# PlasmaControl/spectrogram-enhancement

Measured on AMD Instinct MI355X. Metric: spectrograms/s (STFT+VAE-denoise fwd) at 1/2/4/8 GPUs; PSNR vs CPU ref, higher is better.
Workload: dtype fp16; 1 GPU; BASELINE config 5 per GPU: end-to-end STFT -> SVD -> autoencoder-denoise inference stream, 16,512-sample fp16 shots -> specgr 128x128 (256 hann / hop 128) -> denoiseSignal default -> 3-layer conv AE (16/32/64, 5x5) fp16 forward -> fp16 reconstructions (32,768 B per shot); shots_per_launch=2048, samples=16512, stft_dtype=fp32, svd_dtype=fp32 (fp64 small algebra), ae_dtype=fp16, parallelism=shot-sharded x1, streams_per_gpu=2

## Files before the change

### spectrogram-enhancement_amd/csrc/conv_rows.hip

```cpp
#include <hip/hip_runtime.h>

#include <algorithm>
#include <cstdint>
#include <string>
#include <type_traits>

#include "lds_dma.hpp"
#include "specenh.h"
#include "runtime.hpp"
#include "wave.hpp"

namespace specenh {

namespace {

typedef _Float16 f16x8 __attribute__((ext_vector_type(8)));
typedef __bf16 bf16x8 __attribute__((ext_vector_type(8)));
typedef float f32x4 __attribute__((ext_vector_type(4)));

template <typename T>
__device__ __forceinline__ f32x4 mfma(const uint4& a, const uint4& b, f32x4 acc) {
  if constexpr (__is_same(T, _Float16))
    return __builtin_amdgcn_mfma_f32_16x16x32_f16(__builtin_bit_cast(f16x8, a),
                                                  __builtin_bit_cast(f16x8, b), acc, 0, 0, 0);
// ... 1209 lines not shown
  static constexpr int LDS = RING * ROWB;
  static constexpr int DMA_WAVES = W * CI * 2 / 1024;
  static_assert(WAVES == 4 && DMA_WAVES <= WAVES && (W * CI * 2) % 1024 == 0, "shape");
  static_assert(tap(3, DY0, DY0) || tap(0, DY0, DY0) || any_tap(DY0, 0), "neighbourhood");
};

__device__ __forceinline__ int x32off(int ps, int g) { return ps * 64 + 16 * (g ^ ((ps >> 1) & 3)); }

template <typename T, int CO, int W, int K, int LEAD>
__global__ __launch_bounds__((TC32<CO, W, K>::THREADS)) __attribute__((amdgpu_waves_per_eu(2)))
void convt_rows32_kernel(CRArgs a) {
  using C = TC32<CO, W, K>;
  constexpr int DY0 = C::DY0, DY1 = C::DY1, NDY = C::NDY;
  static_assert(LEAD >= 1 && NDY + LEAD + 1 <= C::RING, "ring: positions g .. g + NDY + LEAD live");
  extern __shared__ __attribute__((aligned(16))) unsigned char ring[];
  const int tid = threadIdx.x, lane = tid & 63;
  const int wv = __builtin_amdgcn_readfirstlane(tid >> 6);
  const int m = lane & 15, kg = lane >> 4;
  const int wx = wv % C::NWIN, nb = wv / C::NWIN;
  const int H = a.H, SPI = H + C::GAP;
  const int G = gridDim.x;
  const int nimg = ((int)a.N - (int)blockIdx.x + G - 1) / G;
  const int S = nimg * SPI;

  {
    uint4* z = reinterpret_cast<uint4*>(ring);
    for (int e = tid; e < C::LDS / 16; e += C::THREADS) z[e] = uint4{0u, 0u, 0u, 0u};
  }
  uint4 wf[K * K];
  {
    const T* __restrict__ Wg = reinterpret_cast<const T*>(a.w);
#pragma unroll
    for (int ph = 0; ph < 4; ++ph)
#pragma unroll
      for (int dy = DY0; dy <= DY1; ++dy)
#pragma unroll
        for (int dx = DY0; dx <= DY1; ++dx)
          if (C::tap(ph, dy, dx))
            wf[C::tap_index(ph, dy, dx)] = *reinterpret_cast<const uint4*>(
                Wg + (((16 * nb + m) * K + C::ky_of(ph >> 1, dy)) * K + C::ky_of(ph & 1, dx)) * 32 +
                8 * kg);
  }
  const f32x4 bias = f32x4{a.b[16 * nb + 4 * kg], a.b[16 * nb + 4 * kg + 1],
                           a.b[16 * nb + 4 * kg + 2], a.b[16 * nb + 4 * kg + 3]};
  resident_loads_landed();
  int xo[NDY];
#pragma unroll
  for (int dx = DY0; dx <= DY1; ++dx) xo[dx - DY0] = x32off(16 * wx + m + dx - DY0, kg);
  const T* __restrict__ X = reinterpret_cast<const T*>(a.x);
  const bool dma_wave = wv < C::DMA_WAVES;
  int dsrc = 0;
  if (dma_wave) {
    const int c = 64 * wv + lane;
    const int x = c / 4, gs = c & 3, ps = x - DY0;
    dsrc = x * 32 + 8 * (gs ^ ((ps >> 1) & 3));
  }
  auto stage_at = [&](int p, int il, int r) -> bool {
    if (!dma_wave) return false;
    unsigned char* dst = ring + (p & 7) * C::ROWB + (-DY0) * 64 + 1024 * wv;
    if (il < nimg && r >= 0 && r < H) {
      const long long n = (long long)blockIdx.x + (long long)il * G;
      lds_dma16_s(X + ((n * H + r) * W) * 32, 2u * dsrc, dst);
      return true;
    }
    *reinterpret_cast<uint4*>(dst + 16 * lane) = uint4{0u, 0u, 0u, 0u};
    return false;
  };
  auto stage = [&](int p) -> bool {
    const int il = p / SPI;
    return stage_at(p, il, p - il * SPI + DY0);
  };
  __syncthreads();
#pragma unroll
  for (int p = 0; p < NDY + LEAD; ++p) stage(p);
  asm volatile("s_waitcnt vmcnt(0)" ::: "memory");
  lds_barrier();

  T* __restrict__ O = reinterpret_cast<T*>(a.out);
  const int OW = 2 * W;
  uint2 pk[4];
  long long po = 0;
  bool held = false;
  int vmn = 0;
  int mk[LEAD + 1];
#pragma unroll
  for (int i = 0; i <= LEAD; ++i) mk[i] = -1;
  auto store_held = [&]() {
    if (held) {
#pragma unroll
      for (int ph = 0; ph < 4; ++ph)
        gstore8(O + po + ((ph >> 1) * OW + (ph & 1)) * CO, pk[ph]);
      vmn += 4;
    }
  };
  int il = 0, s = 0;
  int ilp = (NDY + LEAD) / SPI, sp = NDY + LEAD - ilp * SPI;
  for (int g = 0; g < S; ++g) {
    store_held();
    held = false;
    mk[LEAD] = stage_at(g + NDY + LEAD, ilp, sp + DY0) ? ++vmn : -1;
    if (s < H) {
      f32x4 acc[4] = {bias, bias, bias, bias};
#pragma unroll
      for (int dy = DY0; dy <= DY1; ++dy) {
        const unsigned char* src = ring + ((g + dy - DY0) & 7) * C::ROWB;
#pragma unroll
        for (int dx = DY0; dx <= DY1; ++dx) {
          if (!C::any_tap(dy, dx)) continue;
          const uint4 b = *reinterpret_cast<const uint4*>(src + xo[dx - DY0]);
#pragma unroll
          for (int ph = 0; ph < 4; ++ph)
            if (C::tap(ph, dy, dx)) acc[ph] = mfma<T>(wf[C::tap_index(ph, dy, dx)], b, acc[ph]);
        }
      }
#pragma unroll
      for (int ph = 0; ph < 4; ++ph) pk[ph] = relu_pack4<T>(acc[ph]);
      const long long n = (long long)blockIdx.x + (long long)il * G;
      po = ((n * 2 * H + 2 * s) * OW + 2 * (16 * wx + m)) * CO + 16 * nb + 4 * kg;
      held = true;
    }
    if (mk[0] >= 0) wait_vmcnt_ss<15>(vmn - mk[0]);
    lds_barrier();
#pragma unroll
    for (int i = 0; i < LEAD; ++i) mk[i] = mk[i + 1];
    if (++s == SPI) { s = 0; ++il; }
    if (++sp == SPI) { sp = 0; ++ilp; }
  }
  store_held();
}

template <typename T, int CO, int W, int K>
hipError_t launch_convt_rows32(const CRArgs& a, hipStream_t st) {
  using C = TC32<CO, W, K>;
  constexpr int LEAD = 8 - C::NDY - 1 < 3 ? 8 - C::NDY - 1 : 3;
  const void* k = reinterpret_cast<const void*>(&convt_rows32_kernel<T, CO, W, K, LEAD>);
  static int per_cu[64] = {};
  int dev = 0;
  hipError_t e = hipGetDevice(&dev);
  if (e != hipSuccess) return e;
  if (dev < 0 || dev >= 64) dev = 0;
  if (per_cu[dev] == 0) {
    int pc = 0;
    e = hipOccupancyMaxActiveBlocksPerMultiprocessor(&pc, k, C::THREADS, C::LDS);
    if (e != hipSuccess) return e;
    per_cu[dev] = std::max(1, pc);
  }
  const long long grid = std::min<long long>(a.N, (long long)per_cu[dev] * device_cus());
  SPECENH_LAUNCH((convt_rows32_kernel<T, CO, W, K, LEAD>), dim3((unsigned)grid),
                 dim3(C::THREADS), C::LDS, st, a);
  return hipGetLastError();
}

constexpr int C1W = 128;
constexpr int C1CW = 72;
constexpr int C1ROW = 2 * C1CW;
constexpr int C1RING = 16;
constexpr int C1LDS = C1RING * C1ROW * 4;

template <typename T>
__global__ __launch_bounds__(256) void conv1_rows_pool_kernel(CRArgs a) {
  extern __shared__ __attribute__((aligned(16))) unsigned char ring_raw[];
  uint32_t* const ring = reinterpret_cast<uint32_t*>(ring_raw);
  const int tid = threadIdx.x, lane = tid & 63;
  const int wv = __builtin_amdgcn_readfirstlane(tid >> 6);
  const int m = lane & 15, kg = lane >> 4;
  const int H = a.H, SPI = H / 2 + 2, PPI = H + 4;
  const int G = gridDim.x;
  const int nimg = ((int)a.N - (int)blockIdx.x + G - 1) / G;
  const int S = nimg * SPI;

  for (int e = tid; e < C1RING * C1ROW; e += 256) ring[e] = 0u;
  uint4 w0, w1;
  {
    const T* __restrict__ Wg = reinterpret_cast<const T*>(a.w);
    uint32_t q0[4], q1[4];
#pragma unroll
    for (int i = 0; i < 4; ++i) {
      float v[4];
#pragma unroll
      for (int h = 0; h < 2; ++h) {
        const int kx = 2 * i + h;
        v[2 * h] = kx < 5 ? (float)Wg[(m * 5 + kg) * 5 + kx] : 0.f;
        v[2 * h + 1] = kx < 5 && kg == 0 ? (float)Wg[(m * 5 + 4) * 5 + kx] : 0.f;
      }
      q0[i] = pack2<T>(v[0], v[2]);
      q1[i] = pack2<T>(v[1], v[3]);
    }
    w0 = uint4{q0[0], q0[1], q0[2], q0[3]};
    w1 = uint4{q1[0], q1[1], q1[2], q1[3]};
  }
  const f32x4 bias = f32x4{a.b[4 * kg], a.b[4 * kg + 1], a.b[4 * kg + 2], a.b[4 * kg + 3]};

  const T* __restrict__ X = reinterpret_cast<const T*>(a.x);
  auto stage = [&](int pp) -> int {
    if (wv != 0) return 0;
    int nd = 0;
#pragma unroll
    for (int j = 0; j < 2; ++j) {
      const int pos = pp + j;
      const int il = pos / PPI, r = pos - il * PPI - 2;
      uint32_t* dst = ring + (pos & (C1RING - 1)) * C1ROW + 4;
      if (il < nimg && r >= 0 && r < H) {
        const long long n = (long long)blockIdx.x + (long long)il * G;
        if (lane < 16) lds_dma16(X + (n * H + r) * C1W + 8 * lane, dst);
        ++nd;
      } else if (lane < 16) {
        *reinterpret_cast<uint4*>(dst + 4 * lane) = uint4{0u, 0u, 0u, 0u};
      }
    }
    return nd;
  };
  auto shift = [&](int pp) {
    if (tid < 2 * C1CW) {
      const int j = tid / C1CW, i = tid - j * C1CW;
      uint32_t* row = ring + ((pp + j) & (C1RING - 1)) * C1ROW;
      const uint32_t lo = row[i], hi = row[i + 1];
      row[C1CW + i] = __builtin_amdgcn_alignbit(hi, lo, 16);
    }
  };
  __syncthreads();
  for (int pp = 0; pp < 10; pp += 2) stage(pp);
  asm volatile("s_waitcnt vmcnt(0)" ::: "memory");
  lds_barrier();
  shift(0); shift(2); shift(4);
  lds_barrier();

  const int wbase = 16 * wv + m + 3;
  auto bfrag = [&](int pos, int cb) -> uint4 {
    const uint32_t* row = ring + ((pos + kg) & (C1RING - 1)) * C1ROW + cb * C1CW + wbase;
    return uint4{row[0], row[1], row[2], row[3]};
  };
  T* __restrict__ O = reinterpret_cast<T*>(a.out);
  const int PW = C1W / 2, PH = H / 2;
  for (int g = 0; g < S; ++g) {
    const int nd = stage(2 * g + 10);
    shift(2 * g + 6);
    const int il = g / SPI, p = g - il * SPI;
    if (p < PH) {
      const int pb = 2 * g;
      f32x4 acc[2][2];
#pragma unroll
      for (int dy = 0; dy < 2; ++dy)
#pragma unroll
        for (int cb = 0; cb < 2; ++cb) {
          const uint4 b = bfrag(pb + dy, cb);
          uint4 b4 = bfrag(pb + dy + 4, cb);
          if (kg != 0) b4 = uint4{0u, 0u, 0u, 0u};
          acc[dy][cb] = mfma<T>(w0, b, bias);
          acc[dy][cb] = mfma<T>(w1, b4, acc[dy][cb]);
        }
      float v[4];
#pragma unroll
      for (int i = 0; i < 4; ++i)
        v[i] = fmaxf(fmaxf(fmaxf(acc[0][0][i], acc[0][1][i]), fmaxf(acc[1][0][i], acc[1][1][i])),
                     0.f);
      const long long n = (long long)blockIdx.x + (long long)il * G;
      *reinterpret_cast<uint2*>(O + ((n * PH + p) * PW + 16 * wv + m) * 16 + 4 * kg) =
          uint2{pack2<T>(v[0], v[1]), pack2<T>(v[2], v[3])};
    }
    if (wv == 0) {
      const int younger = nd + (p < PH ? 1 : 0);
      if (younger == 0) asm volatile("s_waitcnt vmcnt(0)" ::: "memory");
      else if (younger == 1) asm volatile("s_waitcnt vmcnt(1)" ::: "memory");
      else if (younger == 2) asm volatile("s_waitcnt vmcnt(2)" ::: "memory");
      else asm volatile("s_waitcnt vmcnt(3)" ::: "memory");
    }
    lds_barrier();
  }
}

template <typename T>
hipError_t launch_conv1_rows(const CRArgs& a, hipStream_t st) {
  const void* k = reinterpret_cast<const void*>(&conv1_rows_pool_kernel<T>);
  static int per_cu[64] = {};
  int dev = 0;
  hipError_t e = hipGetDevice(&dev);
  if (e != hipSuccess) return e;
  if (dev < 0 || dev >= 64) dev = 0;
  if (per_cu[dev] == 0) {
    int pc = 0;
    e = hipOccupancyMaxActiveBlocksPerMultiprocessor(&pc, k, 256, C1LDS);
    if (e != hipSuccess) return e;
    per_cu[dev] = std::max(1, pc);
  }
  const long long grid = std::min<long long>(a.N, (long long)per_cu[dev] * device_cus());
  SPECENH_LAUNCH(conv1_rows_pool_kernel<T>, dim3((unsigned)grid), dim3(256), C1LDS, st, a);
  return hipGetLastError();
}

struct E2Args {
  const void* x;
  const void* w1;
  const float* b1;
  const void* w2;
  const float* b2;
  void* out;
  int N, H;
};

constexpr int E2R1 = 32;
#ifndef SPECENH_ENC2_COPIES
#define SPECENH_ENC2_COPIES 4
#endif
constexpr int E2NC = SPECENH_ENC2_COPIES;
__host__ __device__ constexpr int E2CB(int c) {
  return E2NC == 4 ? (c == 0 ? 0 : c == 1 ? 72 : c == 2 ? 178 : 250) : c * C1CW;
}
constexpr int E2ROW = E2NC == 4 ? 352 : 2 * C1CW;
constexpr int E2RROWS = E2R1 + 2;
#ifndef SPECENH_ENC2_STAGGER
#define SPECENH_ENC2_STAGGER 0
#endif

constexpr int E2LDS = RC<16, 32, 64>::LDS + E2RROWS * E2ROW * 4 + 48 * 4;
constexpr int E2TILE = 32 * 32 * 2;
constexpr int E2LDS1 = E2LDS + 2 * E2TILE;
__host__ __device__ constexpr int e2_tile_write(int p, int c8) {
  return 64 * p + 8 * (c8 ^ (2 * ((p >> 1) & 3)));
}
__host__ __device__ constexpr int e2_tile_read(int k, int l) {
  const int p = 16 * k + (l >> 2);
  return 64 * p + 16 * ((l & 3) ^ ((p >> 1) & 3));
}

__device__ __forceinline__ uint32_t max_s16x2(uint32_t x, uint32_t y) {
  typedef short s2 __attribute__((ext_vector_type(2)));
  return __builtin_bit_cast(uint32_t, __builtin_elementwise_max(__builtin_bit_cast(s2, x),
                                                                __builtin_bit_cast(s2, y)));
}

template <typename T, int WPE, int SCHED = 0>
__global__ __launch_bounds__(512) __attribute__((amdgpu_waves_per_eu(WPE)))
void enc2_rows_kernel(E2Args a) {
  static_assert(SCHED == 0 || (SCHED == 1 && WPE == 4), "schedule");
  using C = RC<16, 32, 64>;
  extern __shared__ __attribute__((aligned(16))) unsigned char lds[];
  unsigned char* const ring = lds;
  uint32_t* const ring1 = reinterpret_cast<uint32_t*>(lds + C::LDS);
  const int tid = threadIdx.x, lane = tid & 63;
  const int wv = __builtin_amdgcn_readfirstlane(tid >> 6);
  const int m = lane & 15, kg = lane >> 4;
  const int wx = wv % C::NWIN, nb = wv / C::NWIN;
  const int x0 = 16 * wx;
  const int H1 = a.H, H = H1 / 2;
  const int SPI = H / 2 + 1, PPI = H1 + 4;
  const int G = gridDim.x;
  const int nimg = ((int)a.N - (int)blockIdx.x + G - 1) / G;
  const int S = nimg * SPI + 1;

  for (int e = tid; e < (C::LDS + E2RROWS * E2ROW * 4) / 16; e += 512)
    reinterpret_cast<uint4*>(lds)[e] = uint4{0u, 0u, 0u, 0u};
  float* const btab = reinterpret_cast<float*>(lds + C::LDS + E2RROWS * E2ROW * 4);
  if (tid < 16) btab[tid] = a.b1[tid];
  else if (tid < 48) btab[tid] = a.b2[tid - 16];
  auto bias2_ld = [&]() { return *reinterpret_cast<const f32x4*>(btab + 16 + 16 * nb + 4 * kg); };

  uint4 wf[13];
  {
    const T* __restrict__ Wg = reinterpret_cast<const T*>(a.w2);
    const int co = 16 * nb + m, hi = kg >> 1, c8 = 8 * (kg & 1);
    auto tap = [&](int ky, int kx) {
      return *reinterpret_cast<const uint4*>(Wg + ((co * 5 + ky) * 5 + kx) * 16 + c8);
    };
#pragma unroll
    for (int ky = 0; ky < 5; ++ky) {
      wf[ky] = tap(ky, hi);
      wf[5 + ky] = tap(ky, 2 + hi);
    }
    wf[10] = tap(hi, 4);
    wf[11] = tap(2 + hi, 4);
    wf[12] = hi ? uint4{0u, 0u, 0u, 0u} : tap(4, 4);
  }

  const int boff = (x0 + m + (kg >> 1)) * 32 + 16 * (kg & 1);
  const int fo = (x0 + m + 4) * 32 + 16 * (kg & 1);
  const int foff = fo + (kg >> 1) * C::ROWB, foffw = fo - (kg >> 1) * 7 * C::ROWB;

  uint4 v0, v1;
  {
    const T* __restrict__ W1 = reinterpret_cast<const T*>(a.w1);
    uint32_t q0[4], q1[4];
#pragma unroll
    for (int i = 0; i < 4; ++i) {
      float v[4];
#pragma unroll
      for (int h = 0; h < 2; ++h) {
        const int kx = 2 * i + h;
        v[2 * h] = kx < 5 ? (float)W1[(m * 5 + kg) * 5 + kx] : 0.f;
        v[2 * h + 1] = kx < 5 && kg == 0 ? (float)W1[(m * 5 + 4) * 5 + kx] : 0.f;
      }
      q0[i] = pack2<T>(v[0], v[2]);
      q1[i] = pack2<T>(v[1], v[3]);
    }
    v0 = uint4{q0[0], q0[1], q0[2], q0[3]};
    v1 = uint4{q1[0], q1[1], q1[2], q1[3]};
  }
  resident_loads_landed();
  const int w1x = wv & 3, jr = wv >> 2;
  const int wbase = 16 * w1x + m + 3;
  const int p1 = 16 * w1x + m;
  const int c4hi = 2 * ((p1 + 3) & 1), w4 = p1 + 3 - ((p1 + 3) & 1);
  const int cbase0 = E2CB(c4hi) + w4, cbase1 = E2CB(1 + c4hi) + w4;

  const T* __restrict__ X = reinterpret_cast<const T*>(a.x);
  auto stage1_at = [&](int pos, int il, int y) -> int {
    uint32_t* dst = ring1 + (pos & (E2R1 - 1)) * E2ROW + 4;
    if (il < nimg && y >= 0 && y < H1) {
      const long long n = (long long)blockIdx.x + (long long)il * G;
      if (lane < 16) lds_dma16_s(X + (n * H1 + y) * C1W, 16u * lane, dst);
      return 1;
    }
    int z = 0;
    asm volatile("" : "+v"(z));
    if (lane < 16) *reinterpret_cast<uint4*>(dst + 4 * lane) = uint4{(uint32_t)z, (uint32_t)z, (uint32_t)z, (uint32_t)z};
    return 0;
  };
  auto stage1 = [&](int pp) -> int {
    if (wv >= 4) return 0;
    const int pos = pp + wv;
    const int il = pos / PPI;
    return stage1_at(pos, il, pos - il * PPI - 2);
  };
  auto shift1 = [&](int pp) {
    constexpr int NW = E2NC == 4 ? C1CW - 2 : C1CW;
    if (tid < 4 * NW) {
      const int j = tid / NW, i = tid - j * NW;
      uint32_t* row = ring1 + ((pp + j) & (E2R1 - 1)) * E2ROW;
      const uint32_t r0 = row[i], r1 = row[i + 1];
      row[E2CB(1) + i] = __builtin_amdgcn_alignbit(r1, r0, 16);
      if constexpr (E2NC == 4) {
        const uint32_t r2 = row[i + 2];
        row[E2CB(2) + i] = r1;
        row[E2CB(3) + i] = __builtin_amdgcn_alignbit(r2, r1, 16);
      }
    }
  };
  auto run_at = [&](const uint32_t* row, int cb) -> uint4 {
    if constexpr (E2NC == 4) {
      typedef __attribute__((address_space(3))) const volatile unsigned long long lds_u64;
      const lds_u64* r = (const lds_u64*)(row + (cb ? cbase1 : cbase0));
      const unsigned long long lo = r[0], hi = r[1];
      return uint4{(uint32_t)lo, (uint32_t)(lo >> 32), (uint32_t)hi, (uint32_t)(hi >> 32)};
    } else {
      const uint32_t* r = row + cb * C1CW + wbase;
      return uint4{r[0], r[1], r[2], r[3]};
    }
  };
  auto bfrag = [&](int pos, int cb) -> uint4 {
    return run_at(ring1 + ((pos + kg) & (E2R1 - 1)) * E2ROW, cb);
  };
  auto bfrag4 = [&](int pos, int cb) -> uint4 {
    const uint32_t* zrow = ring1 + (E2NC == 4 ? E2R1 + 1 - (pos & 1) : E2R1) * E2ROW;
    return run_at(kg == 0 ? ring1 + (pos & (E2R1 - 1)) * E2ROW : zrow, cb);
  };
  auto produce = [&](int g2, int il, int q2) {
    const int r = 2 * q2 + jr;
    const int pb = 4 * g2 + 2 * jr;
    float v[4] = {0.f, 0.f, 0.f, 0.f};
    const f32x4 bias1 = *reinterpret_cast<const f32x4*>(btab + 4 * kg);
#pragma unroll
    for (int dy = 0; dy < 2; ++dy)
#pragma unroll
      for (int cb = 0; cb < 2; ++cb) {
        const uint4 b = bfrag(pb + dy, cb);
        const uint4 b4 = bfrag4(pb + dy + 4, cb);
        f32x4 acc1 = mfma<T>(v0, b, bias1);
        acc1 = mfma<T>(v1, b4, acc1);
#pragma unroll
        for (int i = 0; i < 4; ++i) v[i] = fmaxf(v[i], acc1[i]);
      }
    const bool real = il < nimg && r < H;
    const uint2 pk = real ? uint2{pack2<T>(v[0], v[1]), pack2<T>(v[2], v[3])} : uint2{0u, 0u};
    *reinterpret_cast<uint2*>(ring + ((2 * g2 + jr) & 7) * C::ROWB + (16 * w1x + m + 2) * 32 +
                              8 * kg) = pk;
  };

  __syncthreads();
  for (int pp = 0; pp < 32; pp += 4) stage1(pp);
  asm volatile("s_waitcnt vmcnt(0)" ::: "memory");
  lds_barrier();
  for (int pp = 0; pp < 16; pp += 4) shift1(pp);
  lds_barrier();
  produce(0, 0, 0);
  produce(1, 1 / SPI, 1 % SPI);
  lds_barrier();

  f32x4 acc[6];
#pragma unroll
  for (int i = 0; i < 6; ++i) acc[i] = bias2_ld();
  T* __restrict__ O = reinterpret_cast<T*>(a.out);
  const int PW = 32, PHh = H / 2;
  int c_1 = 0, c_2 = 0;
  auto fdiv = [](int x, int d) { return x >= 0 ? x / d : -((-x + d - 1) / d); };
  int ilA = fdiv(-2, SPI), qA = -2 - ilA * SPI;
  int qC = 0;
  int ilB = 2 / SPI, qB = 2 - ilB * SPI;
  int ilD = (32 + wv) / PPI, rD = 32 + wv - ilD * PPI;
  auto adv = [](int& il, int& q, int by, int per) {
    q += by;
    if (q >= per) { q -= per; ++il; }
  };
#ifdef SPECENH_CR_STATS
  CRClock clk;
#endif

  if constexpr (SCHED == 1) {
    unsigned char* const tile = lds + E2LDS;
    unsigned char* const tw = tile + e2_tile_write((x0 + m) >> 1, 4 * nb + kg);
    auto store_tile = [&](unsigned char* base, int tb) {
      int l = lane;
      asm volatile("" : "+v"(l));
      const uint4 v = *reinterpret_cast<const uint4*>(tile + tb + e2_tile_read(wv & 1, l));
      gstore16_s<0>(base, 1024u * (wv & 1) + 16u * l, v);
    };
    const int nimgs = __builtin_amdgcn_readfirstlane(nimg);
    ilD = __builtin_amdgcn_readfirstlane(ilD);
    rD = __builtin_amdgcn_readfirstlane(rD);
    constexpr unsigned E2F_REAL = 1u, E2F_BUB = 2u, E2F_TOP = 4u;
    constexpr unsigned F_PROD = E2F_REAL, F_CBUB = E2F_BUB << 6, F_CTOP = E2F_TOP << 6,
                       F_OTOP = E2F_TOP << 12, F_HELD = E2F_REAL << 15;
    int ilT = 0, qT = 0;
    unsigned fl = 0;
    auto lt = [](int x, int y) -> unsigned { return (unsigned)(x - y) >> 31; };
    auto push = [&]() {
      const unsigned in = lt(qT, PHh);
      fl = (fl << 3) | ((lt(ilT, nimgs) & in) * E2F_REAL) | ((in ^ 1u) * E2F_BUB) |
           (lt(qT, 1) * E2F_TOP);
    };
    auto walk = [&]() {
      if (++qT == SPI) { qT = 0; ++ilT; }
    };
    push();
    walk();
    push();
    walk();
    push();
    fl = __builtin_amdgcn_readfirstlane(fl);
    constexpr long long ROWO = E2TILE;
    unsigned char* ob = reinterpret_cast<unsigned char*>(a.out) +
                        (((long long)blockIdx.x - G) * PHh + SPI - 2) * ROWO;
    unsigned char* obp = ob - ROWO;
    const long long ojump = (long long)(G - 1) * PHh * ROWO;
    constexpr long long ROWX = (long long)C1W * (long long)sizeof(T);
    const unsigned char* xs = reinterpret_cast<const unsigned char*>(a.x) +
        (((long long)blockIdx.x + (long long)ilD * G) * H1 + rD - 2) * ROWX;
    const long long xjump = (long long)(G - 1) * H1 * ROWX;
    const int zr = wv < 2 ? wv : H1 + wv;
    auto dma_real = [&]() { return lt(ilD, nimgs) & (lt(rD, zr) | lt(zr, rD)); };
    unsigned dreal = __builtin_amdgcn_readfirstlane(dma_real());
    auto next = [&]() {
      walk();
      push();
      obp = ob;
      ob += (fl & F_OTOP) ? ojump : ROWO;
      rD += 4;
      if (rD >= PPI) { rD -= PPI; ++ilD; xs += xjump; } else { xs += 4 * ROWX; }
      dreal = __builtin_amdgcn_readfirstlane(dma_real());
      fl = __builtin_amdgcn_readfirstlane(fl);
      asm volatile("" : "+s"(fl), "+s"(dreal), "+s"(ob), "+s"(obp), "+s"(xs));
    };
    auto ld16 = [](const unsigned char* p) { return *reinterpret_cast<const uint4*>(p); };
    struct Pair { uint4 b, b4; };
    auto c1_read = [&](int pb, int pr) {
      return Pair{bfrag(pb + (pr >> 1), pr & 1), bfrag4(pb + (pr >> 1) + 4, pr & 1)};
    };
    auto c1_max = [&](float (&v)[4], const f32x4& acc1) {
#pragma unroll
      for (int i = 0; i < 4; ++i) v[i] = fmaxf(v[i], acc1[i]);
    };

    auto step1 = [&](auto ic, const int s) {
      constexpr int I = decltype(ic)::value % 3, P = decltype(ic)::value & 1;
      auto slot = [](int d) { return (2 * I + d + 12) % 6; };
      const unsigned flc = fl;
      f32x4& r0 = acc[slot(-4)];
      f32x4& r1 = acc[slot(-3)];
      if (wv >= 6 && (flc & F_HELD)) store_tile(obp, (P ^ 1) * E2TILE);
      CR_MARK(0);
      int nd = 0;
      if (wv < 4) {
        uint32_t* dst = ring1 + ((4 * s + wv) & (E2R1 - 1)) * E2ROW + 4;
        if (dreal) {
          if (lane < 16) lds_dma16_s(xs, 16u * lane, dst);
          nd = 1;
        } else {
          int z = 0;
          asm volatile("" : "+v"(z));
          if (lane < 16) *reinterpret_cast<uint4*>(dst + 4 * lane) = uint4{(uint32_t)z, (uint32_t)z, (uint32_t)z, (uint32_t)z};
        }
      }
      shift1(4 * s + 16);
      CR_MARK(1);
      const int rs = (2 * s) & 7;
      const unsigned char* rb = ring + rs * C::ROWB;
      const int pb = 4 * (s + 2) + 2 * jr;
      const int fo1 = (flc & F_CBUB) ? 0 : (rs + 1) * C::ROWB + (rs == 6 && kg >= 2 ? foff - 8 * C::ROWB : foff);
      const int foT = (flc & F_CTOP) && kg >= 2 ? (rs - 1) * C::ROWB + foff : 0;
      float v[4] = {0.f, 0.f, 0.f, 0.f};
      auto c2 = [&](int j, int w, const uint4& b) {
        const int d = w < 10 ? j + 2 - w % 5 : w == 10 ? j + 2 : w == 11 ? j : j - 2;
        acc[slot(d)] = mfma<T>(wf[w], b, acc[slot(d)]);
      };
      const f32x4 bias1 = *reinterpret_cast<const f32x4*>(btab + 4 * kg);
      auto c1a = [&](const Pair& f) { return mfma<T>(v0, f.b, bias1); };
      auto c1b = [&](const Pair& f, const f32x4& a1) { return mfma<T>(v1, f.b4, a1); };
      {
        auto nbr = [](uint32_t x) {
          return (uint32_t)__builtin_amdgcn_update_dpp(0, (int)x, 0xB1, 0xF, 0xF, true);
        };
        const uint32_t p0 = max_s16x2(pack2<T>(r0[0], r0[1]), pack2<T>(r1[0], r1[1]));
        const uint32_t p1 = max_s16x2(pack2<T>(r0[2], r0[3]), pack2<T>(r1[2], r1[3]));
        const f32x4 bias = bias2_ld();
        r0 = bias;
        r1 = bias;
        *reinterpret_cast<uint2*>(tw + P * E2TILE) =
            uint2{max_s16x2(max_s16x2(p0, nbr(p0)), 0u), max_s16x2(max_s16x2(p1, nbr(p1)), 0u)};
      }
      next();
#pragma unroll
      for (int pr = 0; pr < 4; ++pr) {
        const Pair f = c1_read(pb, pr);
        c1_max(v, c1b(f, c1a(f)));
      }
      CR_MARK(2);
#pragma unroll
      for (int j = 0; j < 2; ++j) {
        const unsigned char* rbj = rb + j * C::ROWB;
        const uint4 b0 = ld16(rbj + boff), b2 = ld16(rbj + boff + 64);
        const uint4 bF = j ? ld16(ring + fo1) : ld16(rbj + foff);
#pragma unroll
        for (int w = 0; w < 5; ++w) c2(j, w, b0);
#pragma unroll
        for (int w = 5; w < 10; ++w) c2(j, w, b2);
        c2(j, 10, bF); c2(j, 11, bF); c2(j, 12, bF);
        if (j == 0) acc[slot(1)] = mfma<T>(wf[10], ld16(ring + foT), acc[slot(1)]);
      }
      {
        const uint2 pv = uint2{pack2<T>(v[0], v[1]), pack2<T>(v[2], v[3])};
        const uint32_t keep = 0u - (flc & F_PROD);
        *reinterpret_cast<uint2*>(ring + ((2 * s + 4 + jr) & 7) * C::ROWB + (16 * w1x + m + 2) * 32 +
                                  8 * kg) = uint2{pv.x & keep, pv.y & keep};
      }
      CR_MARK(3);
      if (wv < 4) wait_vmcnt_ss<3>(c_2 + c_1 + nd);
      c_2 = c_1;
      c_1 = nd;
      CR_MARK(4);
      lds_barrier();
      CR_MARK(5);
    };
    const int Ss = __builtin_amdgcn_readfirstlane(S);
    CR_MARK(-1);
    for (int s = 0; s < Ss; s += 6) {
      step1(std::integral_constant<int, 0>{}, s);
      if (s + 1 >= Ss) break;
      step1(std::integral_constant<int, 1>{}, s + 1);
      if (s + 2 >= Ss) break;
      step1(std::integral_constant<int, 2>{}, s + 2);
      if (s + 3 >= Ss) break;
      step1(std::integral_constant<int, 3>{}, s + 3);
      if (s + 4 >= Ss) break;
      step1(std::integral_constant<int, 4>{}, s + 4);
      if (s + 5 >= Ss) break;
      step1(std::integral_constant<int, 5>{}, s + 5);
    }
    if (wv >= 6 && (fl & F_HELD)) store_tile(obp, ((Ss - 1) & 1) * E2TILE);
#ifdef SPECENH_CR_STATS
    clk.flush(wv);
#endif
    return;
  }

  auto step = [&](auto ic, const int s) {
    constexpr int I = decltype(ic)::value;
    auto slot = [](int d) { return (2 * I + d + 12) % 6; };
    int ns = 0;
    {
      f32x4& r0 = acc[slot(-4)];
      f32x4& r1 = acc[slot(-3)];
      {
        const int il = ilA, q = qA;
        if (il >= 0 && il < nimg && q < PHh) {
          ns = 1;
          float v[4];
#pragma unroll
          for (int i = 0; i < 4; ++i) v[i] = fmaxf(max_pair(fmaxf(r0[i], r1[i])), 0.f);
          const long long n = (long long)blockIdx.x + (long long)il * G;
          const long long o = ((n * PHh + q) * PW + (x0 + m) / 2) * 32 + 16 * nb + 4 * kg;
          *reinterpret_cast<uint2*>(O + o) = uint2{pack2<T>(v[0], v[1]), pack2<T>(v[2], v[3])};
        }
      }
      const f32x4 bias = bias2_ld();
      r0 = bias;
      r1 = bias;
    }
    CR_MARK(0);
    const int nd = wv < 4 ? stage1_at(4 * s + 32 + wv, ilD, rD - 2) : 0;
    shift1(4 * s + 16);
    CR_MARK(1);
    const int q = qC;
    auto conv2_rows = [&]() {
#pragma unroll
    for (int j = 0; j < 2; ++j) {
      const int rs = (2 * s + j) & 7;
      const unsigned char* rb = ring + rs * C::ROWB;
      const uint4 b0 = *reinterpret_cast<const uint4*>(rb + boff);
      const uint4 b2 = *reinterpret_cast<const uint4*>(rb + boff + 64);
      uint4 bF = *reinterpret_cast<const uint4*>(rb + (rs == 7 ? foffw : foff));
      if (j == 1 && q == SPI - 1) bF = uint4{0u, 0u, 0u, 0u};
#pragma unroll
      for (int ky = 0; ky < 5; ++ky) {
        f32x4& ac = acc[slot(j + 2 - ky)];
        ac = mfma<T>(wf[ky], b0, ac);
      }
#pragma unroll
      for (int ky = 0; ky < 5; ++ky) {
        f32x4& ac = acc[slot(j + 2 - ky)];
        ac = mfma<T>(wf[5 + ky], b2, ac);
      }
      acc[slot(j + 2)] = mfma<T>(wf[10], bF, acc[slot(j + 2)]);
      acc[slot(j)] = mfma<T>(wf[11], bF, acc[slot(j)]);
      acc[slot(j - 2)] = mfma<T>(wf[12], bF, acc[slot(j - 2)]);
      if (j == 0) {
        uint4 bT = *reinterpret_cast<const uint4*>(ring + ((2 * s) & 7) * C::ROWB + fo);
        if (kg < 2 || q != 0) bT = uint4{0u, 0u, 0u, 0u};
        acc[slot(1)] = mfma<T>(wf[10], bT, acc[slot(1)]);
      }
    }
    };
    if (SPECENH_ENC2_STAGGER && wv >= 4) {
      conv2_rows();
      produce(s + 2, ilB, qB);
    } else {
      produce(s + 2, ilB, qB);
      CR_MARK(2);
      conv2_rows();
    }
    CR_MARK(3);
    if (wv < 4) {
      const int younger = c_2 + c_1 + ns + nd;
      if (younger >= 6) {
        asm volatile("s_waitcnt vmcnt(6)" ::: "memory");
      } else switch (younger) {
        case 0: asm volatile("s_waitcnt vmcnt(0)" ::: "memory"); break;
        case 1: asm volatile("s_waitcnt vmcnt(1)" ::: "memory"); break;
        case 2: asm volatile("s_waitcnt vmcnt(2)" ::: "memory"); break;
        case 3: asm volatile("s_waitcnt vmcnt(3)" ::: "memory"); break;
        case 4: asm volatile("s_waitcnt vmcnt(4)" ::: "memory"); break;
        case 5: asm volatile("s_waitcnt vmcnt(5)" ::: "memory"); break;
        default: asm volatile("s_waitcnt vmcnt(6)" ::: "memory"); break;
      }
    }
    c_2 = c_1;
    c_1 = ns + nd;
    adv(ilA, qA, 1, SPI);
    qC = qC + 1 == SPI ? 0 : qC + 1;
    adv(ilB, qB, 1, SPI);
    adv(ilD, rD, 4, PPI);
    CR_MARK(4);
    lds_barrier();
    CR_MARK(5);
  };
  CR_MARK(-1);
  int s = 0;
  for (; s + 3 <= S; s += 3) {
    step(std::integral_constant<int, 0>{}, s);
    step(std::integral_constant<int, 1>{}, s + 1);
    step(std::integral_constant<int, 2>{}, s + 2);
  }
  if (s < S) step(std::integral_constant<int, 0>{}, s);
  if (s + 1 < S) step(std::integral_constant<int, 1>{}, s + 1);
#ifdef SPECENH_CR_STATS
  clk.flush(wv);
#endif
}

template <typename T, int WPE, int SCHED>
hipError_t launch_enc2_wpe(const E2Args& a, hipStream_t st) {
  constexpr int LDSB = SCHED == 1 ? E2LDS1 : E2LDS;
  const void* k = reinterpret_cast<const void*>(&enc2_rows_kernel<T, WPE, SCHED>);
  static int per_cu[64] = {};
  int dev = 0;
  hipError_t e = hipGetDevice(&dev);
  if (e != hipSuccess) return e;
  if (dev < 0 || dev >= 64) dev = 0;
  if (per_cu[dev] == 0) {
    int pc = 0;
    e = hipOccupancyMaxActiveBlocksPerMultiprocessor(&pc, k, 512, LDSB);
    if (e != hipSuccess) return e;
    per_cu[dev] = std::max(1, pc);
  }
  const long long grid = std::min<long long>(a.N, (long long)per_cu[dev] * device_cus());
  SPECENH_LAUNCH((enc2_rows_kernel<T, WPE, SCHED>), dim3((unsigned)grid), dim3(512), LDSB, st, a);
  return hipGetLastError();
}

template <typename T>
hipError_t launch_enc2(const E2Args& a, hipStream_t st) {
  if (variant(V_ENC2_WPE2)) return launch_enc2_wpe<T, 2, 0>(a, st);
  if (variant(V_ENC2_SCHED) != 0 && ((uintptr_t)a.out & 15) == 0) return launch_enc2_wpe<T, 4, 1>(a, st);
  return launch_enc2_wpe<T, 4, 0>(a, st);
}

}

int conv_rows_pool(int dtype, const void* x, int N, int H, int W, int CI, const void* w,
                   const float* b, int CO, int K, void* out, hipStream_t st, bool* launched) {
  *launched = false;
  if (variant(V_CONV_NO_ROWS) != 0 || N <= 0 || H < 2 || (H & 1) || !b) return SPECENH_OK;
  if ((long long)N * H * W * CI >= (1ll << 31)) return SPECENH_OK;
  CRArgs a{};
  a.x = x; a.w = w; a.b = b; a.out = out; a.N = N; a.H = H;
  hipError_t e = hipSuccess;
  const bool f16 = dtype == SPECENH_DTYPE_F16;
  if (dtype != SPECENH_DTYPE_F16 && dtype != SPECENH_DTYPE_BF16) return SPECENH_OK;
  if (CI == 16 && CO == 32 && W == 64 && K == 5)
    e = f16 ? launch_rows<_Float16, 16, 32, 64>(a, st) : launch_rows<__bf16, 16, 32, 64>(a, st);
  else if (CI == 32 && CO == 64 && W == 32 && K == 5 && variant(V_CONV_ROWS_SCHED) != 0)
    e = f16 ? launch_rows<_Float16, 32, 64, 32, 5, 1>(a, st) : launch_rows<__bf16, 32, 64, 32, 5, 1>(a, st);
  else if (CI == 32 && CO == 64 && W == 32 && K == 5)
    e = f16 ? launch_rows<_Float16, 32, 64, 32>(a, st) : launch_rows<__bf16, 32, 64, 32>(a, st);
  else if (CI == 32 && CO == 32 && W == 64 && K == 5)
    e = f16 ? launch_rows<_Float16, 32, 32, 64>(a, st) : launch_rows<__bf16, 32, 32, 64>(a, st);
  else if (CI == 32 && CO == 32 && W == 64 && K == 3)
    e = f16 ? launch_rows<_Float16, 32, 32, 64, 3>(a, st) : launch_rows<__bf16, 32, 32, 64, 3>(a, st);
  else
    return SPECENH_OK;
  if (e != hipSuccess) return set_error(SPECENH_EHIP, std::string("conv_rows: ") + hipGetErrorString(e));
  *launched = true;
  return SPECENH_OK;
}

}

namespace specenh {

int convt_rows(int dtype, const void* x, int N, int H, int W, int CI, const void* w,
               const float* b, int CO, int K, void* out, hipStream_t st, bool* launched) {
  *launched = false;
  if (variant(V_CONVT_NO_ROWS) != 0 || N <= 0 || H <= 0 || !b) return SPECENH_OK;
  if (dtype != SPECENH_DTYPE_F16 && dtype != SPECENH_DTYPE_BF16) return SPECENH_OK;
  if ((long long)N * 4 * H * W * CO >= (1ll << 31)) return SPECENH_OK;
  CRArgs a{};
  a.x = x; a.w = w; a.b = b; a.out = out; a.N = N; a.H = H;
  const bool f16 = dtype == SPECENH_DTYPE_F16;
  hipError_t e;
  if (CI == 32) {
    if (CO != 32 || W != 32) return SPECENH_OK;
    if (K == 3) e = f16 ? launch_convt_rows32<_Float16, 32, 32, 3>(a, st) : launch_convt_rows32<__bf16, 32, 32, 3>(a, st);
    else if (K == 5) e = f16 ? launch_convt_rows32<_Float16, 32, 32, 5>(a, st) : launch_convt_rows32<__bf16, 32, 32, 5>(a, st);
    else if (K == 7) e = f16 ? launch_convt_rows32<_Float16, 32, 32, 7>(a, st) : launch_convt_rows32<__bf16, 32, 32, 7>(a, st);
// ... 86 lines not shown
```

Before: 2.047 million spectrograms/s.

## Repack conv1 weight fragments to drop shifted LDS row copies

Rebuilds the first conv layer's MFMA A-fragments so that the 5x5 filter's column offset is folded into two weight variants (cb=0/1) instead of keeping half-word-shifted copies of each input row in LDS. The per-step shift passes (alignbit copies plus barriers) in both the standalone conv1 kernel and the fused enc2 kernel are removed, and each output pair now needs one B-fragment read per row and half as many MFMAs. The fifth kernel row is packed into the fourth B word through a separate k4 row/word lookup. This shrinks the LDS ring and removes the copy traffic, but relies on unusual fragment indexing and wraparound arithmetic that must stay correct.

```diff
diff --git a/spectrogram-enhancement_amd/csrc/conv_rows.hip b/spectrogram-enhancement_amd/csrc/conv_rows.hip
--- a/spectrogram-enhancement_amd/csrc/conv_rows.hip
+++ b/spectrogram-enhancement_amd/csrc/conv_rows.hip
@@ -1385,10 +1385,36 @@
 }
 
 constexpr int C1W = 128;
-constexpr int C1CW = 72;
-constexpr int C1ROW = 2 * C1CW;
+constexpr int C1ROW = 80;
+constexpr int C1ZW = 72;
 constexpr int C1RING = 16;
 constexpr int C1LDS = C1RING * C1ROW * 4;
+
+template <typename T>
+__device__ __forceinline__ uint4 c1_afrag(const T* __restrict__ Wg, int m, int g, int cb) {
+  uint32_t q[4];
+#pragma unroll
+  for (int i = 0; i < 4; ++i) {
+    float v[2];
+#pragma unroll
+    for (int h = 0; h < 2; ++h) {
+      const int j = 2 * i + h;
+      const int ky = j < 6 ? g : 4, c = (j < 6 ? j : 2 * g + j - 6) - cb;
+      v[h] = (j < 6 || g < 3) && c >= 0 && c <= 4 ? (float)Wg[(m * 5 + ky) * 5 + c] : 0.f;
+    }
+    q[i] = pack2<T>(v[0], v[1]);
+  }
+  return uint4{q[0], q[1], q[2], q[3]};
+}
+__device__ __forceinline__ int c1_k4row(int w, int g) { return g < 3 ? 4 : 3 + (w & 1); }
+__device__ __forceinline__ int c1_k4word(int p, int g) { return g < 3 ? p + 3 + g : C1ZW; }
+typedef __attribute__((address_space(3))) const volatile uint32_t c1_lds_u32;
+__device__ __forceinline__ uint4 c1_bfrag(const uint32_t* run, const uint32_t* k4) {
+  c1_lds_u32* r = (c1_lds_u32*)run;
+  c1_lds_u32* r4 = (c1_lds_u32*)k4;
+  const uint32_t a = r[0], b = r[1], c = r[2], d = r4[0];
+  return uint4{a, b, c, d};
+}
 
 template <typename T>
 __global__ __launch_bounds__(256) void conv1_rows_pool_kernel(CRArgs a) {
@@ -1403,25 +1429,8 @@
   const int S = nimg * SPI;
 
   for (int e = tid; e < C1RING * C1ROW; e += 256) ring[e] = 0u;
-  uint4 w0, w1;
-  {
-    const T* __restrict__ Wg = reinterpret_cast<const T*>(a.w);
-    uint32_t q0[4], q1[4];
-#pragma unroll
-    for (int i = 0; i < 4; ++i) {
-      float v[4];
-#pragma unroll
-      for (int h = 0; h < 2; ++h) {
-        const int kx = 2 * i + h;
-        v[2 * h] = kx < 5 ? (float)Wg[(m * 5 + kg) * 5 + kx] : 0.f;
-        v[2 * h + 1] = kx < 5 && kg == 0 ? (float)Wg[(m * 5 + 4) * 5 + kx] : 0.f;
-      }
-      q0[i] = pack2<T>(v[0], v[2]);
-      q1[i] = pack2<T>(v[1], v[3]);
-    }
-    w0 = uint4{q0[0], q0[1], q0[2], q0[3]};
-    w1 = uint4{q1[0], q1[1], q1[2], q1[3]};
-  }
+  const uint4 w0 = c1_afrag<T>(reinterpret_cast<const T*>(a.w), m, kg, 0);
+  const uint4 w1 = c1_afrag<T>(reinterpret_cast<const T*>(a.w), m, kg, 1);
   const f32x4 bias = f32x4{a.b[4 * kg], a.b[4 * kg + 1], a.b[4 * kg + 2], a.b[4 * kg + 3]};
 
   const T* __restrict__ X = reinterpret_cast<const T*>(a.x);
@@ -1443,45 +1452,30 @@
     }
     return nd;
   };
-  auto shift = [&](int pp) {
-    if (tid < 2 * C1CW) {
-      const int j = tid / C1CW, i = tid - j * C1CW;
-      uint32_t* row = ring + ((pp + j) & (C1RING - 1)) * C1ROW;
-      const uint32_t lo = row[i], hi = row[i + 1];
-      row[C1CW + i] = __builtin_amdgcn_alignbit(hi, lo, 16);
-    }
-  };
   __syncthreads();
   for (int pp = 0; pp < 10; pp += 2) stage(pp);
   asm volatile("s_waitcnt vmcnt(0)" ::: "memory");
   lds_barrier();
-  shift(0); shift(2); shift(4);
-  lds_barrier();
 
   const int wbase = 16 * wv + m + 3;
-  auto bfrag = [&](int pos, int cb) -> uint4 {
-    const uint32_t* row = ring + ((pos + kg) & (C1RING - 1)) * C1ROW + cb * C1CW + wbase;
-    return uint4{row[0], row[1], row[2], row[3]};
+  const int k4r = c1_k4row(wv, kg), k4w = c1_k4word(16 * wv + m, kg);
+  auto bfrag = [&](int pos) -> uint4 {
+    return c1_bfrag(ring + ((pos + kg) & (C1RING - 1)) * C1ROW + wbase,
+                    ring + ((pos + k4r) & (C1RING - 1)) * C1ROW + k4w);
   };
   T* __restrict__ O = reinterpret_cast<T*>(a.out);
   const int PW = C1W / 2, PH = H / 2;
   for (int g = 0; g < S; ++g) {
     const int nd = stage(2 * g + 10);
-    shift(2 * g + 6);
     const int il = g / SPI, p = g - il * SPI;
     if (p < PH) {
       const int pb = 2 * g;
+      const uint4 b0 = bfrag(pb), b1 = bfrag(pb + 1);
       f32x4 acc[2][2];
-#pragma unroll
-      for (int dy = 0; dy < 2; ++dy)
-#pragma unroll
-        for (int cb = 0; cb < 2; ++cb) {
-          const uint4 b = bfrag(pb + dy, cb);
-          uint4 b4 = bfrag(pb + dy + 4, cb);
-          if (kg != 0) b4 = uint4{0u, 0u, 0u, 0u};
-          acc[dy][cb] = mfma<T>(w0, b, bias);
-          acc[dy][cb] = mfma<T>(w1, b4, acc[dy][cb]);
-        }
+      acc[0][0] = mfma<T>(w0, b0, bias);
+      acc[0][1] = mfma<T>(w1, b0, bias);
+      acc[1][0] = mfma<T>(w0, b1, bias);
+      acc[1][1] = mfma<T>(w1, b1, bias);
       float v[4];
 #pragma unroll
       for (int i = 0; i < 4; ++i)
@@ -1532,20 +1526,11 @@
 };
 
 constexpr int E2R1 = 32;
-#ifndef SPECENH_ENC2_COPIES
-#define SPECENH_ENC2_COPIES 4
-#endif
-constexpr int E2NC = SPECENH_ENC2_COPIES;
-__host__ __device__ constexpr int E2CB(int c) {
-  return E2NC == 4 ? (c == 0 ? 0 : c == 1 ? 72 : c == 2 ? 178 : 250) : c * C1CW;
-}
-constexpr int E2ROW = E2NC == 4 ? 352 : 2 * C1CW;
-constexpr int E2RROWS = E2R1 + 2;
 #ifndef SPECENH_ENC2_STAGGER
 #define SPECENH_ENC2_STAGGER 0
 #endif
 
-constexpr int E2LDS = RC<16, 32, 64>::LDS + E2RROWS * E2ROW * 4 + 48 * 4;
+constexpr int E2LDS = RC<16, 32, 64>::LDS + E2R1 * C1ROW * 4 + 48 * 4;
 constexpr int E2TILE = 32 * 32 * 2;
 constexpr int E2LDS1 = E2LDS + 2 * E2TILE;
 __host__ __device__ constexpr int e2_tile_write(int p, int c8) {
@@ -1581,9 +1566,9 @@
   const int nimg = ((int)a.N - (int)blockIdx.x + G - 1) / G;
   const int S = nimg * SPI + 1;
 
-  for (int e = tid; e < (C::LDS + E2RROWS * E2ROW * 4) / 16; e += 512)
+  for (int e = tid; e < (C::LDS + E2R1 * C1ROW * 4) / 16; e += 512)
     reinterpret_cast<uint4*>(lds)[e] = uint4{0u, 0u, 0u, 0u};
-  float* const btab = reinterpret_cast<float*>(lds + C::LDS + E2RROWS * E2ROW * 4);
+  float* const btab = reinterpret_cast<float*>(lds + C::LDS + E2R1 * C1ROW * 4);
   if (tid < 16) btab[tid] = a.b1[tid];
   else if (tid < 48) btab[tid] = a.b2[tid - 16];
   auto bias2_ld = [&]() { return *reinterpret_cast<const f32x4*>(btab + 16 + 16 * nb + 4 * kg); };
@@ -1609,35 +1594,16 @@
   const int fo = (x0 + m + 4) * 32 + 16 * (kg & 1);
   const int foff = fo + (kg >> 1) * C::ROWB, foffw = fo - (kg >> 1) * 7 * C::ROWB;
 
-  uint4 v0, v1;
-  {
-    const T* __restrict__ W1 = reinterpret_cast<const T*>(a.w1);
-    uint32_t q0[4], q1[4];
-#pragma unroll
-    for (int i = 0; i < 4; ++i) {
-      float v[4];
-#pragma unroll
-      for (int h = 0; h < 2; ++h) {
-        const int kx = 2 * i + h;
-        v[2 * h] = kx < 5 ? (float)W1[(m * 5 + kg) * 5 + kx] : 0.f;
-        v[2 * h + 1] = kx < 5 && kg == 0 ? (float)W1[(m * 5 + 4) * 5 + kx] : 0.f;
-      }
-      q0[i] = pack2<T>(v[0], v[2]);
-      q1[i] = pack2<T>(v[1], v[3]);
-    }
-    v0 = uint4{q0[0], q0[1], q0[2], q0[3]};
-    v1 = uint4{q1[0], q1[1], q1[2], q1[3]};
-  }
+  const uint4 v0 = c1_afrag<T>(reinterpret_cast<const T*>(a.w1), m, kg, 0);
+  const uint4 v1 = c1_afrag<T>(reinterpret_cast<const T*>(a.w1), m, kg, 1);
   resident_loads_landed();
   const int w1x = wv & 3, jr = wv >> 2;
-  const int wbase = 16 * w1x + m + 3;
-  const int p1 = 16 * w1x + m;
-  const int c4hi = 2 * ((p1 + 3) & 1), w4 = p1 + 3 - ((p1 + 3) & 1);
-  const int cbase0 = E2CB(c4hi) + w4, cbase1 = E2CB(1 + c4hi) + w4;
+  const uint32_t boA = (kg * C1ROW + 16 * w1x + m + 3) * 4;
+  const uint32_t boK = (c1_k4row(w1x, kg) * C1ROW + c1_k4word(16 * w1x + m, kg)) * 4;
 
   const T* __restrict__ X = reinterpret_cast<const T*>(a.x);
   auto stage1_at = [&](int pos, int il, int y) -> int {
-    uint32_t* dst = ring1 + (pos & (E2R1 - 1)) * E2ROW + 4;
+    uint32_t* dst = ring1 + (pos & (E2R1 - 1)) * C1ROW + 4;
     if (il < nimg && y >= 0 && y < H1) {
       const long long n = (long long)blockIdx.x + (long long)il * G;
       if (lane < 16) lds_dma16_s(X + (n * H1 + y) * C1W, 16u * lane, dst);
@@ -1654,54 +1620,28 @@
     const int il = pos / PPI;
     return stage1_at(pos, il, pos - il * PPI - 2);
   };
-  auto shift1 = [&](int pp) {
-    constexpr int NW = E2NC == 4 ? C1CW - 2 : C1CW;
-    if (tid < 4 * NW) {
-      const int j = tid / NW, i = tid - j * NW;
-      uint32_t* row = ring1 + ((pp + j) & (E2R1 - 1)) * E2ROW;
-      const uint32_t r0 = row[i], r1 = row[i + 1];
-      row[E2CB(1) + i] = __builtin_amdgcn_alignbit(r1, r0, 16);
-      if constexpr (E2NC == 4) {
-        const uint32_t r2 = row[i + 2];
-        row[E2CB(2) + i] = r1;
-        row[E2CB(3) + i] = __builtin_amdgcn_alignbit(r2, r1, 16);
-      }
-    }
-  };
-  auto run_at = [&](const uint32_t* row, int cb) -> uint4 {
-    if constexpr (E2NC == 4) {
-      typedef __attribute__((address_space(3))) const volatile unsigned long long lds_u64;
-      const lds_u64* r = (const lds_u64*)(row + (cb ? cbase1 : cbase0));
-      const unsigned long long lo = r[0], hi = r[1];
-      return uint4{(uint32_t)lo, (uint32_t)(lo >> 32), (uint32_t)hi, (uint32_t)(hi >> 32)};
-    } else {
-      const uint32_t* r = row + cb * C1CW + wbase;
-      return uint4{r[0], r[1], r[2], r[3]};
-    }
-  };
-  auto bfrag = [&](int pos, int cb) -> uint4 {
-    return run_at(ring1 + ((pos + kg) & (E2R1 - 1)) * E2ROW, cb);
-  };
-  auto bfrag4 = [&](int pos, int cb) -> uint4 {
-    const uint32_t* zrow = ring1 + (E2NC == 4 ? E2R1 + 1 - (pos & 1) : E2R1) * E2ROW;
-    return run_at(kg == 0 ? ring1 + (pos & (E2R1 - 1)) * E2ROW : zrow, cb);
+  auto bfrag = [&](int pos) -> uint4 {
+    constexpr uint32_t RB = E2R1 * C1ROW * 4;
+    const uint32_t sb = (uint32_t)(pos & (E2R1 - 1)) * (C1ROW * 4);
+    const uint32_t oA = sb + boA, oK = sb + boK;
+    const unsigned char* r1b = reinterpret_cast<const unsigned char*>(ring1);
+    return c1_bfrag(reinterpret_cast<const uint32_t*>(r1b + min(oA, oA - RB)),
+                    reinterpret_cast<const uint32_t*>(r1b + min(oK, oK - RB)));
+  };
+  auto c1_window = [&](float (&v)[4], const uint4& bA, const uint4& bB, const f32x4& bias1) {
+#pragma unroll
+    for (int pr = 0; pr < 4; ++pr) {
+      const f32x4 acc1 = mfma<T>(pr & 1 ? v1 : v0, pr >> 1 ? bB : bA, bias1);
+#pragma unroll
+      for (int i = 0; i < 4; ++i) v[i] = fmaxf(v[i], acc1[i]);
+    }
   };
   auto produce = [&](int g2, int il, int q2) {
     const int r = 2 * q2 + jr;
     const int pb = 4 * g2 + 2 * jr;
     float v[4] = {0.f, 0.f, 0.f, 0.f};
-    const f32x4 bias1 = *reinterpret_cast<const f32x4*>(btab + 4 * kg);
-#pragma unroll
-    for (int dy = 0; dy < 2; ++dy)
-#pragma unroll
-      for (int cb = 0; cb < 2; ++cb) {
-        const uint4 b = bfrag(pb + dy, cb);
-        const uint4 b4 = bfrag4(pb + dy + 4, cb);
-        f32x4 acc1 = mfma<T>(v0, b, bias1);
-        acc1 = mfma<T>(v1, b4, acc1);
-#pragma unroll
-        for (int i = 0; i < 4; ++i) v[i] = fmaxf(v[i], acc1[i]);
-      }
+    const uint4 bA = bfrag(pb), bB = bfrag(pb + 1);
+    c1_window(v, bA, bB, *reinterpret_cast<const f32x4*>(btab + 4 * kg));
     const bool real = il < nimg && r < H;
     const uint2 pk = real ? uint2{pack2<T>(v[0], v[1]), pack2<T>(v[2], v[3])} : uint2{0u, 0u};
     *reinterpret_cast<uint2*>(ring + ((2 * g2 + jr) & 7) * C::ROWB + (16 * w1x + m + 2) * 32 +
@@ -1711,8 +1651,6 @@
   __syncthreads();
   for (int pp = 0; pp < 32; pp += 4) stage1(pp);
   asm volatile("s_waitcnt vmcnt(0)" ::: "memory");
-  lds_barrier();
-  for (int pp = 0; pp < 16; pp += 4) shift1(pp);
   lds_barrier();
   produce(0, 0, 0);
   produce(1, 1 / SPI, 1 % SPI);
@@ -1793,14 +1731,6 @@
       asm volatile("" : "+s"(fl), "+s"(dreal), "+s"(ob), "+s"(obp), "+s"(xs));
     };
     auto ld16 = [](const unsigned char* p) { return *reinterpret_cast<const uint4*>(p); };
-    struct Pair { uint4 b, b4; };
-    auto c1_read = [&](int pb, int pr) {
-      return Pair{bfrag(pb + (pr >> 1), pr & 1), bfrag4(pb + (pr >> 1) + 4, pr & 1)};
-    };
-    auto c1_max = [&](float (&v)[4], const f32x4& acc1) {
-#pragma unroll
-      for (int i = 0; i < 4; ++i) v[i] = fmaxf(v[i], acc1[i]);
-    };
 
     auto step1 = [&](auto ic, const int s) {
       constexpr int I = decltype(ic)::value % 3, P = decltype(ic)::value & 1;
@@ -1812,7 +1742,7 @@
       CR_MARK(0);
       int nd = 0;
       if (wv < 4) {
-        uint32_t* dst = ring1 + ((4 * s + wv) & (E2R1 - 1)) * E2ROW + 4;
+        uint32_t* dst = ring1 + ((4 * s + wv) & (E2R1 - 1)) * C1ROW + 4;
         if (dreal) {
           if (lane < 16) lds_dma16_s(xs, 16u * lane, dst);
           nd = 1;
@@ -1822,11 +1752,11 @@
           if (lane < 16) *reinterpret_cast<uint4*>(dst + 4 * lane) = uint4{(uint32_t)z, (uint32_t)z, (uint32_t)z, (uint32_t)z};
         }
       }
-      shift1(4 * s + 16);
       CR_MARK(1);
       const int rs = (2 * s) & 7;
       const unsigned char* rb = ring + rs * C::ROWB;
       const int pb = 4 * (s + 2) + 2 * jr;
+      const uint4 bA = bfrag(pb), bB = bfrag(pb + 1);
       const int fo1 = (flc & F_CBUB) ? 0 : (rs + 1) * C::ROWB + (rs == 6 && kg >= 2 ? foff - 8 * C::ROWB : foff);
       const int foT = (flc & F_CTOP) && kg >= 2 ? (rs - 1) * C::ROWB + foff : 0;
       float v[4] = {0.f, 0.f, 0.f, 0.f};
@@ -1834,9 +1764,6 @@
         const int d = w < 10 ? j + 2 - w % 5 : w == 10 ? j + 2 : w == 11 ? j : j - 2;
         acc[slot(d)] = mfma<T>(wf[w], b, acc[slot(d)]);
       };
-      const f32x4 bias1 = *reinterpret_cast<const f32x4*>(btab + 4 * kg);
-      auto c1a = [&](const Pair& f) { return mfma<T>(v0, f.b, bias1); };
-      auto c1b = [&](const Pair& f, const f32x4& a1) { return mfma<T>(v1, f.b4, a1); };
       {
         auto nbr = [](uint32_t x) {
           return (uint32_t)__builtin_amdgcn_update_dpp(0, (int)x, 0xB1, 0xF, 0xF, true);
@@ -1850,11 +1777,7 @@
             uint2{max_s16x2(max_s16x2(p0, nbr(p0)), 0u), max_s16x2(max_s16x2(p1, nbr(p1)), 0u)};
       }
       next();
-#pragma unroll
-      for (int pr = 0; pr < 4; ++pr) {
-        const Pair f = c1_read(pb, pr);
-        c1_max(v, c1b(f, c1a(f)));
-      }
+      c1_window(v, bA, bB, *reinterpret_cast<const f32x4*>(btab + 4 * kg));
       CR_MARK(2);
 #pragma unroll
       for (int j = 0; j < 2; ++j) {
@@ -1929,7 +1852,6 @@
     }
     CR_MARK(0);
     const int nd = wv < 4 ? stage1_at(4 * s + 32 + wv, ilD, rD - 2) : 0;
-    shift1(4 * s + 16);
     CR_MARK(1);
     const int q = qC;
     auto conv2_rows = [&]() {
```

Result: faster. 2.099 million spectrograms/s (median of 6 runs) (+2.6%).
